# snayfach/MIDAS

Hardware: AMD Instinct MI355X
Metric: genomic sites/sec pileup+allele-count (higher is better)
Workload: dtype u8/u32 integer tallies (fp64 only in the two keep_read ratio tests)

## Files before the change

### midas_amd/build.py

```python

import concurrent.futures
import os
import shutil
import subprocess
import sys

HERE = os.path.dirname(os.path.abspath(__file__))
CSRC = os.path.join(HERE, "csrc")
LIB_DIR = os.path.join(HERE, "lib")
OBJ_DIR = os.path.join(LIB_DIR, "obj")
LIB_NAME = "libmidas_snps_hip.so"
LIB_PATH = os.path.join(LIB_DIR, LIB_NAME)

SOURCES = ["contigs.cpp", "bgzf_host.cpp", "bam_host.cpp", "bam_shares.cpp", "bam_writer.cpp", "tables_host.cpp", "fasta_host.cpp", "row_deflate.cpp", "comm.cpp", "pack_reads.hip", "index_reads.hip", "pileup_tiles.hip", "index_direct.hip", "pileup_direct.hip", "pileup_long.hip", "rows_deflate.hip", "bgzf_inflate.hip", "bam_walk.hip", "measure.hip", "merge_sites.hip", "merge_rows.hip", "tables_scan.hip", "tables_device.hip", "genes_count.hip", "genes_merge_io.cpp", "genes_merge.hip", "sites_io.cpp", "sites_scan.hip", "sites_strains.hip", "sites_trees.hip", "sites_pairs.hip", "sites_ld.hip", "nj_tree.hip", "genes_compare.hip", "genes_linkage.hip", "sam_scan.hip", "species_hits.hip", "species_assign.cpp", "species_merge.hip", "device_sort.hip", "mt19937_stream.hip", "bam_device.hip", "ctx_runtime.hip", "batch.hip", "batch_direct.hip", "batch_packed.hip", "batch_rows.hip"]
HEADERS = ["layout.h", "contigs.h", "kernels.h", "device_common.h", "pileup_common.h", "direct_common.h", "dense_bases.h", "ctx_internal.h", "batch.h", "filter_tables.h", "work_plan.h", "hostio.h", "hostio_internal.h", "bam_parse.h", "bam_record.h", "decode_plan.h", "sam_resident_plan.h", "tables_plan.h", "row_deflate.h", "workers.h", "crc32.h", "text_numbers.h", "text_rows.h", "bit_planes.h", "row_group_plan.h", "genes_rows.h", "sites_rows.h", "sites_call.h", "sites_resample.h", "draw_plan.h", "pandas_f64.h", "merge_fmt.h", "merge_rows.h", os.path.join("..", "..", "include", "midas_snps.h")]

FLAGS = ["--offload-arch=gfx950", "-O3", "-std=c++17", "-fPIC", "-mllvm", "-amdgpu-atomic-optimizer-strategy=None"]
SOURCE_FLAGS = {"sites_scan.hip": ["-ffp-contract=off"], "sites_strains.hip": ["-ffp-contract=off"], "sites_trees.hip": ["-ffp-contract=off"], "sites_pairs.hip": ["-ffp-contract=off"], "sites_ld.hip": ["-ffp-contract=off"],
                "genes_compare.hip": ["-ffp-contract=off"], "species_hits.hip": ["-ffp-contract=off"],
                "species_assign.cpp": ["-ffp-contract=off"], "species_merge.hip": ["-ffp-contract=off"], "merge_rows.hip": ["-ffp-contract=off"], "nj_tree.hip": ["-ffp-contract=off"]}


def _hipcc():
    for cand in (os.environ.get("HIPCC"), shutil.which("hipcc"), "/opt/rocm/bin/hipcc"):
        if cand and os.path.exists(cand):
            return cand
    raise RuntimeError("hipcc not found: cannot build %s" % LIB_NAME)


def _sources():
    return [s for s in SOURCES if os.path.exists(os.path.join(CSRC, s))]


def _newest_header():
    t = 0.0
    for h in HEADERS:
        p = os.path.join(CSRC, h)
        if os.path.exists(p):
            t = max(t, os.path.getmtime(p))
    return max(t, os.path.getmtime(os.path.abspath(__file__)))


def _stale():
    if not os.path.exists(LIB_PATH):
        return True
    t = os.path.getmtime(LIB_PATH)
    if _newest_header() > t:
        return True
    return any(os.path.getmtime(os.path.join(CSRC, s)) > t for s in _sources())


def _compile(obj, cmd, verbose):
    tmp = obj + ".tmp.%d" % os.getpid()
    try:
        _run(cmd + [tmp], verbose)
        os.replace(tmp, obj)
    finally:
        if os.path.exists(tmp):
            os.unlink(tmp)


def _run(cmd, verbose):
    if verbose:
        print(" ".join(cmd), file=sys.stderr)
    res = subprocess.run(cmd, stdout=subprocess.PIPE, stderr=subprocess.STDOUT, text=True)
    if res.returncode != 0:
        raise RuntimeError("hipcc failed (%d): %s\n%s" % (res.returncode, " ".join(cmd), res.stdout))


def build_native(force=False, verbose=False, extra_flags=(), lib_path=None, replace=None):
    variant = bool(extra_flags) or lib_path is not None or bool(replace)
    out = lib_path or LIB_PATH
    if not force and not variant and not _stale():
        return out
    hipcc = _hipcc()
    obj_dir = OBJ_DIR if not variant else OBJ_DIR + ".variant.%d" % os.getpid()
    os.makedirs(obj_dir, exist_ok=True)
    hdr_t = _newest_header()
    jobs = []
    objs = []
    for s in _sources():
        src = os.path.abspath(replace[s]) if replace and s in replace else os.path.join(CSRC, s)
        obj = os.path.join(obj_dir, s.replace(".", "_") + ".o")
        objs.append(obj)
        if force or variant or not os.path.exists(obj) or os.path.getmtime(obj) < max(hdr_t, os.path.getmtime(src)):
            jobs.append((obj, [hipcc] + FLAGS + SOURCE_FLAGS.get(s, []) + list(extra_flags) + ["-I", CSRC, "-x", "hip", "-c", src, "-o"]))
    try:
        workers = max(1, min(len(jobs), (os.cpu_count() or 4)))
        if jobs:
            with concurrent.futures.ThreadPoolExecutor(max_workers=workers) as pool:
                for f in [pool.submit(_compile, o, j, verbose) for (o, j) in jobs]:
                    f.result()
        tmp = out + ".tmp.%d" % os.getpid()
        try:
            _run([hipcc, "--offload-arch=gfx950", "-shared", "-fPIC"] + objs + ["-o", tmp, "-lz", "-lpthread", "-ldl"], verbose)
            os.replace(tmp, out)
        finally:
            if os.path.exists(tmp):
                os.unlink(tmp)
    finally:
        if variant:
            shutil.rmtree(obj_dir, ignore_errors=True)
    return out


if __name__ == "__main__":
    args = [a for a in sys.argv[1:]]
    force = "--force" in args
    verbose = "-v" in args
    out = None
    extra = []
    repl = {}
    it = iter(a for a in args if a not in ("--force", "-v"))
    for a in it:
        if a == "-o":
            out = next(it)
        elif a == "--replace":
            k, v = next(it).split("=", 1)
            repl[k] = v
        else:
            extra.append(a)
    print(build_native(force=force, verbose=verbose, extra_flags=extra, lib_path=out, replace=repl))
```

### midas_amd/csrc/index_direct.hip

```cpp
#include "dense_bases.h"
#include "direct_common.h"

namespace midas {

using namespace dev;
using namespace direct;

namespace {

constexpr int kIdxBlock = 256;
#ifndef MIDAS_IDX_RUN
#define MIDAS_IDX_RUN 2048
#endif
constexpr int kIdxRun = MIDAS_IDX_RUN;

__device__ __forceinline__ int contig_of_read(const DirectIndexParams& p, int i) {
  int lo = 0, hi = p.n_contigs;
  while (lo < hi) {
    const int mid = (lo + hi) >> 1;
    if (p.contig_read_begin[mid] > i) hi = mid; else lo = mid + 1;
  }
  int c = lo - 1;
  c = c < 0 ? 0 : c;
  return c > p.n_contigs - 1 ? p.n_contigs - 1 : c;
}
struct ContigCursor {
  int c, begin, next_begin, tile_base, tile_end;
  long long clen;
  __device__ __forceinline__ void fetch(const DirectIndexParams& p) {
    begin = p.contig_read_begin[c];
    next_begin = p.contig_read_begin[c + 1];
    clen = p.contig_len[c];
    tile_base = p.contig_tile_base[c];
    tile_end = p.contig_tile_base[c + 1];
  }
  __device__ __forceinline__ void advance(const DirectIndexParams& p, int i) {
    if (i < next_begin || c + 1 >= p.n_contigs) return;
    while (c + 1 < p.n_contigs && i >= p.contig_read_begin[c + 1]) ++c;
    fetch(p);
  }
};

__device__ __forceinline__ unsigned long long block_sum(unsigned long long v, unsigned long long* lds4) {
  for (int d = 32; d >= 1; d >>= 1) v += __shfl_down(v, d);
  __syncthreads();
  if ((threadIdx.x & 63) == 0) lds4[threadIdx.x >> 6] = v;
  __syncthreads();
  return lds4[0] + lds4[1] + lds4[2] + lds4[3];
}
__device__ __forceinline__ unsigned long long block_max(unsigned long long v, unsigned long long* lds4) {
  for (int d = 32; d >= 1; d >>= 1) {
    const unsigned long long o = __shfl_down(v, d);
    v = o > v ? o : v;
  }
  __syncthreads();
  if ((threadIdx.x & 63) == 0) lds4[threadIdx.x >> 6] = v;
  __syncthreads();
  const unsigned long long a = lds4[0] > lds4[1] ? lds4[0] : lds4[1], b = lds4[2] > lds4[3] ? lds4[2] : lds4[3];
  return a > b ? a : b;
}

template <bool SORTED>
__global__ __launch_bounds__(kIdxBlock) void direct_ranges_kernel(DirectIndexParams p) {
  __shared__ int s_c0;
  if (blockIdx.x == 0) {
    for (int i = threadIdx.x; i < p.n_stat_words; i += kIdxBlock) p.stats[i] = 0ull;
    if (threadIdx.x == 0 && p.err) *p.err = kNoError;
  }
  for (int i = blockIdx.x * kIdxBlock + threadIdx.x; i < p.n_tiles; i += gridDim.x * kIdxBlock) {
    p.tbegin_next[i] = 0xFFFFFFFFu;
    p.tend_next[i] = 0u;
  }
  const long long lo = (long long)blockIdx.x * kIdxRun;
  const long long hi = lo + kIdxRun < (long long)p.n_reads ? lo + kIdxRun : (long long)p.n_reads;
  if (lo >= hi) return;
  (void)s_c0;
  ContigCursor cur;
  {
    const DirectBlockCursor bc = p.block_contig[blockIdx.x];
    cur.c = bc.c; cur.begin = bc.begin; cur.next_begin = bc.next_begin; cur.tile_base = bc.tile_base; cur.tile_end = bc.tile_end;
    cur.clen = bc.clen;
  }
  const int lane = threadIdx.x & 63;
  constexpr int U = kIdxRun / kIdxBlock;
  int32_t pos[U], before[U];
#pragma unroll
  for (int u = 0; u < U; ++u) {
    const long long ii = lo + (long long)u * kIdxBlock + threadIdx.x;
    const long long ic = ii < hi ? ii : hi - 1;
    pos[u] = p.pos[ic];
    before[u] = p.pos[ic > 0 ? ic - 1 : 0];
  }
#pragma unroll
  for (int u = 0; u < U; ++u) {
    const long long ii = lo + (long long)u * kIdxBlock + threadIdx.x;
    const bool valid = ii < hi;
    uint32_t key = 0xFFFFFFFEu;
    int ka = 0, kb = 0;
    if (valid) {
      const int i = (int)ii;
      cur.advance(p, i);
      const long long last = cur.clen - 1;
      long long pc = pos[u];
      pc = pc < 0 ? 0 : (pc > last ? last : pc);
      const long long pr = pc + p.reach < last ? pc + p.reach : last;
      ka = cur.tile_base + (int)(pc >> p.tile_shift);
      kb = cur.tile_base + (int)(pr >> p.tile_shift);
      if (SORTED) {
        const bool first_of_contig = i == cur.begin;
        long long pb = before[u];
        pb = pb < 0 ? 0 : (pb > last ? last : pb);
        const long long pbr = pb + p.reach < last ? pb + p.reach : last;
        const int ka0 = first_of_contig ? cur.tile_base : cur.tile_base + (int)(pb >> p.tile_shift);
        const int kb0 = first_of_contig ? cur.tile_base - 1 : cur.tile_base + (int)(pbr >> p.tile_shift);
        for (int t = ka0; t < ka; ++t) p.tend[t] = (uint32_t)i;
        for (int t = kb0 + 1; t <= kb; ++t) p.tbegin[t] = (uint32_t)i;
        if (i == cur.next_begin - 1)
          for (int t = ka; t < cur.tile_end; ++t) p.tend[t] = (uint32_t)i + 1u;
      } else {
        key = (uint32_t)ka;
      }
    }
    if (!SORTED) {
      const uint32_t key_before = __shfl_up(key, 1), key_after = __shfl_down(key, 1);
      if (valid) {
        const uint32_t i = (uint32_t)ii;
        if (lane == 0 || key_before != key) atomicMin(&p.tbegin[ka], i);
        if (lane == 63 || key_after != key) atomicMax(&p.tend[ka], i + 1u);
        for (int t = ka + 1; t <= kb; ++t) {
          atomicMin(&p.tbegin[t], i);
          atomicMax(&p.tend[t], i + 1u);
        }
      }
    }
  }
}

struct Fields {
  long long so, so1, qo, qo1, co, co1;
  int32_t pos, l, nm;
};
__device__ __forceinline__ Fields load_fields(const DirectIndexParams& p, long long i) {
  Fields f;
  f.so = p.seq_off[i]; f.so1 = p.seq_off[i + 1];
  f.qo = p.qual_off[i]; f.qo1 = p.qual_off[i + 1];
  f.co = p.cigar_off[i]; f.co1 = p.cigar_off[i + 1];
  f.pos = p.pos[i]; f.l = p.l_seq[i]; f.nm = p.nm[i];
  return f;
}
__device__ __forceinline__ bool bad_layout(const DirectIndexParams& p, const Fields& f) {
  const long long l = f.l;
  return l < 0 || f.co1 - f.co < 0 || f.co < 0 || f.so < 0 || f.qo < 0 || f.so1 - f.so < (l + 1) / 2 || f.qo1 - f.qo < l ||
         f.so1 > p.seq_bytes || f.qo1 > p.qual_bytes || f.co1 > p.n_cigar;
}

__global__ __launch_bounds__(kIdxBlock) void direct_facts_kernel(DirectIndexParams p) {
  __shared__ unsigned long long red[4];
  __shared__ int s_c0;
  const long long lo = (long long)blockIdx.x * kIdxRun;
  const long long hi = lo + kIdxRun < (long long)p.n_reads ? lo + kIdxRun : (long long)p.n_reads;
  if (threadIdx.x == 0 && lo < hi) {
    s_c0 = contig_of_read(p, (int)lo);
    ContigCursor c0;
    c0.c = s_c0;
    c0.fetch(p);
    DirectBlockCursor bc;
    bc.c = c0.c; bc.begin = c0.begin; bc.next_begin = c0.next_begin; bc.tile_base = c0.tile_base; bc.tile_end = c0.tile_end; bc.pad = 0;
    bc.clen = c0.clen;
    p.block_contig[blockIdx.x] = bc;
  }
  __syncthreads();
  unsigned long long alg = 0, status = kNoError;
  uint32_t maxl = 0, maxspan = 0, unsorted = 0, general = 0, n_long = 0, n_out = 0, maxcommon = 0;
  ContigCursor cur;
  if (lo < hi) {
    cur.c = s_c0;
    cur.fetch(p);
  }
  for (long long ii = lo + threadIdx.x; ii < hi; ii += kIdxBlock) {
    const int i = (int)ii;
    cur.advance(p, i);
    const Fields f = load_fields(p, ii);
    const long long l = f.l, nc = f.co1 - f.co;
    {
      const long long last = cur.clen - 1;
      long long pc = f.pos, pb = p.pos[i > 0 ? i - 1 : 0];
      pc = pc < 0 ? 0 : (pc > last ? last : pc);
      pb = pb < 0 ? 0 : (pb > last ? last : pb);
      if (i != cur.begin && pb > pc) unsorted = 1u;
    }
    if (bad_layout(p, f)) {
      const unsigned long long s = ((unsigned long long)i << 8) | kPackBadLayout;
      status = s < status ? s : status;
      continue;
    }
    alg += (unsigned long long)((l + 1) / 2 + l + 4 * nc + 16);
    maxl = (uint32_t)l > maxl ? (uint32_t)l : maxl;
    if (l > kMaxLSeq || nc > kMaxField16 || f.nm > kMaxField16) {
      n_long += 1u;
      continue;
    }
    CigarView cg;
    cg.load(p.rec ? reinterpret_cast<const uint32_t*>(p.payload + ((unsigned long long)p.rec[i].off8 << 3)) : p.cigar + f.co);
    unsigned long long span = 0;
    for_each_op(cg, (uint32_t)nc, [&](uint32_t, uint32_t v) {
      const uint32_t op = v & 15u;
      if (op_is_match(op) || op == OP_D || op == OP_N) span += (unsigned long long)(v >> 4);
      return true;
    });
    span = span > 0x3FFFFFFFull ? 0x3FFFFFFFull : span;
    maxspan = (uint32_t)span > maxspan ? (uint32_t)span : maxspan;
    if (span > (unsigned long long)p.overhang) {
      n_out += 1u;
      const long long last = cur.clen - 1;
      long long pc = f.pos;
      pc = pc < 0 ? 0 : (pc > last ? last : pc);
      long long e = (long long)f.pos + (long long)span - 1;
      e = e > last ? last : e;
      if (e >= pc) {
        const uint32_t ka = (uint32_t)cur.tile_base + (uint32_t)(pc >> p.tile_shift), kb = (uint32_t)cur.tile_base + (uint32_t)(e >> p.tile_shift);
        if (kb > ka) {
          const uint32_t slot = atomicAdd(p.n_outliers_listed, 1u);
          if (slot < p.outlier_cap) p.outliers[slot] = DirectOutlier{(uint32_t)i, ka + 1u, kb, 0u};
        }
        const long long tile_start = (pc >> p.tile_shift) << p.tile_shift;
        if (e - tile_start >= (long long)(1 << p.tile_shift) + p.overhang)
          for (uint32_t t = ka; t <= kb; ++t) p.tile_flag[t] = 1;
      }
    } else {
      maxcommon = (uint32_t)span > maxcommon ? (uint32_t)span : maxcommon;
    }
    ReadShape sh;
    const bool fast = (uint32_t)nc <= 4u && decode_shape(cg.c0, cg.c1, cg.c2, cg.c3, (uint32_t)nc, (uint32_t)l, &sh) && f.nm >= 0 &&
                      f.pos >= 0 && (long long)f.pos < cur.clen;
    general += fast ? 0u : 1u;
  }
  alg = block_sum(alg, red);
  const unsigned long long ngen = block_sum((unsigned long long)general, red);
  const unsigned long long nlong = block_sum((unsigned long long)n_long, red);
  const unsigned long long bmax = block_max((unsigned long long)maxl, red);
  const unsigned long long bspan = block_max((unsigned long long)maxspan, red);
  const unsigned long long bcommon = block_max((unsigned long long)maxcommon, red);
  const unsigned long long nout = block_sum((unsigned long long)n_out, red);
  const unsigned long long any_unsorted = block_max((unsigned long long)unsorted, red);
  const unsigned long long worst = ~block_max(~status, red);
  if (threadIdx.x == 0) {
    DirectFacts* f = p.facts + (blockIdx.x % kDirectFactSlots);
    if (alg) atomicAdd(&f->alg_bytes, alg);
    if (ngen) atomicAdd(&f->n_general, (uint32_t)ngen);
    if (nlong) atomicAdd(&f->n_long, (uint32_t)nlong);
    if (bmax) atomicMax(&f->max_l, (uint32_t)bmax);
    if (bspan) atomicMax(&f->max_span, (uint32_t)bspan);
    if (bcommon) atomicMax(&f->max_span_common, (uint32_t)bcommon);
    if (nout) atomicAdd(&f->n_outliers, (uint32_t)nout);
    if (any_unsorted) atomicOr(&f->unsorted, 1u);
    if (worst != kNoError) atomicMin(&f->status, worst);
  }
}

__device__ __forceinline__ uint32_t read_units(const DirectLayoutParams& p, long long i) {
  return direct_payload_units((uint32_t)p.l_seq[i], (uint32_t)(p.cigar_off[i + 1] - p.cigar_off[i]));
}

__global__ __launch_bounds__(kIdxBlock) void direct_layout_units_kernel(DirectLayoutParams p) {
  __shared__ unsigned long long red[4];
  const long long lo = (long long)blockIdx.x * kIdxRun;
  const long long hi = lo + kIdxRun < p.n_reads ? lo + kIdxRun : p.n_reads;
  unsigned long long u = 0;
  for (long long i = lo + threadIdx.x; i < hi; i += kIdxBlock) u += read_units(p, i);
  u = block_sum(u, red);
  if (threadIdx.x == 0) p.block_units[blockIdx.x] = u;
}

__global__ __launch_bounds__(kIdxBlock) void direct_layout_scan_kernel(unsigned long long* v, int n_blocks) {
  __shared__ unsigned long long part[kIdxBlock];
  __shared__ unsigned long long carry;
  if (threadIdx.x == 0) carry = 0ull;
  __syncthreads();
  for (int base = 0; base < n_blocks; base += kIdxBlock) {
    const int i = base + (int)threadIdx.x;
    const unsigned long long x = i < n_blocks ? v[i] : 0ull;
    part[threadIdx.x] = x;
    __syncthreads();
    for (int d = 1; d < kIdxBlock; d <<= 1) {
      const unsigned long long y = (int)threadIdx.x >= d ? part[threadIdx.x - d] : 0ull;
      __syncthreads();
      part[threadIdx.x] += y;
      __syncthreads();
    }
    const unsigned long long c = carry;
    if (i < n_blocks) v[i] = c + part[threadIdx.x] - x;
    __syncthreads();
    if (threadIdx.x == kIdxBlock - 1) carry = c + part[kIdxBlock - 1];
    __syncthreads();
  }
  if (threadIdx.x == 0) v[n_blocks] = carry;
}

typedef uint32_t lay_u32x4_a1 __attribute__((ext_vector_type(4), aligned(1)));
__device__ __forceinline__ void group_copy(uint8_t* dst, const uint8_t* src, uint32_t len, int gl) {
  for (uint32_t k = (uint32_t)gl * 16u; k < len; k += 256u) {
    if (k + 16u <= len) {
      *reinterpret_cast<lay_u32x4_a1*>(dst + k) = *reinterpret_cast<const lay_u32x4_a1*>(src + k);
    } else {
      for (uint32_t j = k; j < len; ++j) dst[j] = src[j];
    }
  }
}

__global__ __launch_bounds__(kIdxBlock) void direct_layout_fill_kernel(DirectLayoutParams p) {
  constexpr int U = kIdxRun / kIdxBlock;
  __shared__ uint32_t s_off[kIdxRun];
  __shared__ uint32_t s_part[kIdxBlock];
  const long long lo = (long long)blockIdx.x * kIdxRun;
  const long long hi = lo + kIdxRun < p.n_reads ? lo + kIdxRun : p.n_reads;
  const unsigned long long base = p.block_units[blockIdx.x];
  uint32_t units[U], sum = 0;
#pragma unroll
  for (int u = 0; u < U; ++u) {
    const long long i = lo + (long long)threadIdx.x * U + u;
    units[u] = i < hi ? read_units(p, i) : 0u;
    sum += units[u];
  }
  s_part[threadIdx.x] = sum;
  __syncthreads();
  for (int d = 1; d < kIdxBlock; d <<= 1) {
    const uint32_t y = (int)threadIdx.x >= d ? s_part[threadIdx.x - d] : 0u;
    __syncthreads();
    s_part[threadIdx.x] += y;
    __syncthreads();
  }
  uint32_t run = s_part[threadIdx.x] - sum;
#pragma unroll
  for (int u = 0; u < U; ++u) {
    const long long i = lo + (long long)threadIdx.x * U + u;
    s_off[threadIdx.x * U + u] = run;
    if (i < hi) {
      const int32_t nm = p.nm[i];
      DirectRec r;
      r.pos = p.pos[i];
      r.l_nc = (uint32_t)p.l_seq[i] | ((uint32_t)(p.cigar_off[i + 1] - p.cigar_off[i]) << 16);
      r.nmq = (nm < 0 ? (uint32_t)kNmAbsent : (uint32_t)nm) | ((uint32_t)p.mapq[i] << 16);
      r.off8 = (uint32_t)(base + run);
      p.rec[i] = r;
    }
    run += units[u];
  }
  if (blockIdx.x == gridDim.x - 1 && threadIdx.x == 0) {
    DirectRec r;
    r.pos = 0; r.l_nc = 0u; r.nmq = 0u; r.off8 = (uint32_t)(base + s_part[kIdxBlock - 1]);
    p.rec[p.n_reads] = r;
  }
  __syncthreads();
  const int grp = (int)(threadIdx.x >> 4), gl = (int)(threadIdx.x & 15);
  for (long long i = lo + grp; i < hi; i += kIdxBlock / 16) {
    const uint32_t l = (uint32_t)p.l_seq[i];
    const long long co = p.cigar_off[i];
    const uint32_t nc = (uint32_t)(p.cigar_off[i + 1] - co);
    uint8_t* dst = p.payload + 8ull * (base + s_off[(int)(i - lo)]);
    group_copy(dst, reinterpret_cast<const uint8_t*>(p.cigar + co), 4u * nc, gl);
    (void)dense::encode<16>(dst + 4u * nc, 8u * direct_payload_units(l, nc) - 4u * nc, p.seq4 + p.seq_off[i], p.qual + p.qual_off[i], l, gl, p.side);
  }
}

__global__ __launch_bounds__(256) void direct_outliers_kernel(const DirectOutlier* list, uint32_t n, uint32_t* tbegin) {
  const uint32_t j = blockIdx.x * 256u + threadIdx.x;
  if (j >= n) return;
  const DirectOutlier o = list[j];
  for (uint32_t t = o.t_first; t <= o.t_last; ++t) atomicMin(&tbegin[t], o.read);
}

}

hipError_t launch_direct_outliers(const DirectOutlier* list, uint32_t n, uint32_t* tbegin, hipStream_t s) {
  if (n == 0u) return hipSuccess;
  hipLaunchKernelGGL(direct_outliers_kernel, dim3((n + 255u) / 256u), dim3(256), 0, s, list, n, tbegin);
  return hipGetLastError();
}

int direct_index_blocks(int64_t n_reads) { return n_reads > 0 ? (int)((n_reads + kIdxRun - 1) / kIdxRun) : 1; }

hipError_t launch_direct_facts(const DirectIndexParams& p, hipStream_t s) {
  hipLaunchKernelGGL(direct_facts_kernel, dim3(direct_index_blocks(p.n_reads)), dim3(kIdxBlock), 0, s, p);
  return hipGetLastError();
}

hipError_t launch_direct_layout_sizes(const DirectLayoutParams& p, hipStream_t s) {
  const int nb = direct_index_blocks(p.n_reads);
  hipLaunchKernelGGL(direct_layout_units_kernel, dim3(nb), dim3(kIdxBlock), 0, s, p);
  hipLaunchKernelGGL(direct_layout_scan_kernel, dim3(1), dim3(kIdxBlock), 0, s, p.block_units, nb);
  return hipGetLastError();
}

hipError_t launch_direct_layout_fill(const DirectLayoutParams& p, hipStream_t s) {
  hipLaunchKernelGGL(direct_layout_fill_kernel, dim3(direct_index_blocks(p.n_reads)), dim3(kIdxBlock), 0, s, p);
  return hipGetLastError();
}

hipError_t launch_direct_ranges(const DirectIndexParams& p, hipStream_t s) {
  const int grid = direct_index_blocks(p.n_reads);
  if (p.sorted) hipLaunchKernelGGL(direct_ranges_kernel<true>, dim3(grid), dim3(kIdxBlock), 0, s, p);
  else hipLaunchKernelGGL(direct_ranges_kernel<false>, dim3(grid), dim3(kIdxBlock), 0, s, p);
  return hipGetLastError();
}

}
```

Baseline: 114.4 billion.

## Restructure sorted tile-range indexing with vectorized lane-contiguous loads and ballot-skipped stores

The sorted path of the direct ranges kernel is rewritten so each lane owns four consecutive reads, loaded with a single 16-byte vector load. The previous read's position now comes from a cross-lane shuffle instead of a second global load. Wave-uniform contig fields are hoisted with readfirstlane when a block covers a single contig. A wave ballot skips the store loops when no lane has tile boundaries to publish, and the tile math moves to 32-bit arithmetic. The intent is to cut redundant global loads and divergent per-read work in a small indexing pre-pass, at the cost of more complex lane geometry and an extra head-element load per group.

Result: slower. 110.8 billion (-3.1%).

```diff
diff --git a/midas_amd/build.py b/midas_amd/build.py
--- a/midas_amd/build.py
+++ b/midas_amd/build.py
@@ -13,7 +13,7 @@
 LIB_PATH = os.path.join(LIB_DIR, LIB_NAME)
 
 SOURCES = ["contigs.cpp", "bgzf_host.cpp", "bam_host.cpp", "bam_shares.cpp", "bam_writer.cpp", "tables_host.cpp", "fasta_host.cpp", "row_deflate.cpp", "comm.cpp", "pack_reads.hip", "index_reads.hip", "pileup_tiles.hip", "index_direct.hip", "pileup_direct.hip", "pileup_long.hip", "rows_deflate.hip", "bgzf_inflate.hip", "bam_walk.hip", "measure.hip", "merge_sites.hip", "merge_rows.hip", "tables_scan.hip", "tables_device.hip", "genes_count.hip", "genes_merge_io.cpp", "genes_merge.hip", "sites_io.cpp", "sites_scan.hip", "sites_strains.hip", "sites_trees.hip", "sites_pairs.hip", "sites_ld.hip", "nj_tree.hip", "genes_compare.hip", "genes_linkage.hip", "sam_scan.hip", "species_hits.hip", "species_assign.cpp", "species_merge.hip", "device_sort.hip", "mt19937_stream.hip", "bam_device.hip", "ctx_runtime.hip", "batch.hip", "batch_direct.hip", "batch_packed.hip", "batch_rows.hip"]
-HEADERS = ["layout.h", "contigs.h", "kernels.h", "device_common.h", "pileup_common.h", "direct_common.h", "dense_bases.h", "ctx_internal.h", "batch.h", "filter_tables.h", "work_plan.h", "hostio.h", "hostio_internal.h", "bam_parse.h", "bam_record.h", "decode_plan.h", "sam_resident_plan.h", "tables_plan.h", "row_deflate.h", "workers.h", "crc32.h", "text_numbers.h", "text_rows.h", "bit_planes.h", "row_group_plan.h", "genes_rows.h", "sites_rows.h", "sites_call.h", "sites_resample.h", "draw_plan.h", "pandas_f64.h", "merge_fmt.h", "merge_rows.h", os.path.join("..", "..", "include", "midas_snps.h")]
+HEADERS = ["layout.h", "contigs.h", "kernels.h", "device_common.h", "pileup_common.h", "direct_common.h", "ranges_tiles.h", "dense_bases.h", "ctx_internal.h", "batch.h", "filter_tables.h", "work_plan.h", "hostio.h", "hostio_internal.h", "bam_parse.h", "bam_record.h", "decode_plan.h", "sam_resident_plan.h", "tables_plan.h", "row_deflate.h", "workers.h", "crc32.h", "text_numbers.h", "text_rows.h", "bit_planes.h", "row_group_plan.h", "genes_rows.h", "sites_rows.h", "sites_call.h", "sites_resample.h", "draw_plan.h", "pandas_f64.h", "merge_fmt.h", "merge_rows.h", os.path.join("..", "..", "include", "midas_snps.h")]
 
 FLAGS = ["--offload-arch=gfx950", "-O3", "-std=c++17", "-fPIC", "-mllvm", "-amdgpu-atomic-optimizer-strategy=None"]
 SOURCE_FLAGS = {"sites_scan.hip": ["-ffp-contract=off"], "sites_strains.hip": ["-ffp-contract=off"], "sites_trees.hip": ["-ffp-contract=off"], "sites_pairs.hip": ["-ffp-contract=off"], "sites_ld.hip": ["-ffp-contract=off"],
diff --git a/midas_amd/csrc/index_direct.hip b/midas_amd/csrc/index_direct.hip
--- a/midas_amd/csrc/index_direct.hip
+++ b/midas_amd/csrc/index_direct.hip
@@ -1,5 +1,6 @@
 #include "dense_bases.h"
 #include "direct_common.h"
+#include "ranges_tiles.h"
 
 namespace midas {
 
@@ -9,10 +10,12 @@
 namespace {
 
 constexpr int kIdxBlock = 256;
-#ifndef MIDAS_IDX_RUN
-#define MIDAS_IDX_RUN 2048
+
+#ifdef MIDAS_ISA_MARKS
+#define MIDAS_MARK(name) asm volatile("; MARK " name)
+#else
+#define MIDAS_MARK(name) do { } while (0)
 #endif
-constexpr int kIdxRun = MIDAS_IDX_RUN;
 
 __device__ __forceinline__ int contig_of_read(const DirectIndexParams& p, int i) {
   int lo = 0, hi = p.n_contigs;
@@ -60,9 +63,7 @@
   return a > b ? a : b;
 }
 
-template <bool SORTED>
-__global__ __launch_bounds__(kIdxBlock) void direct_ranges_kernel(DirectIndexParams p) {
-  __shared__ int s_c0;
+__device__ __forceinline__ void reset_for_the_next_run(const DirectIndexParams& p) {
   if (blockIdx.x == 0) {
     for (int i = threadIdx.x; i < p.n_stat_words; i += kIdxBlock) p.stats[i] = 0ull;
     if (threadIdx.x == 0 && p.err) *p.err = kNoError;
@@ -71,10 +72,121 @@
     p.tbegin_next[i] = 0xFFFFFFFFu;
     p.tend_next[i] = 0u;
   }
+}
+
+constexpr int kLaneReads = kRangesLaneReads;
+constexpr int kGroupReads = kIdxBlock * kLaneReads;
+constexpr int kGroups = kIdxRun / kGroupReads;
+static_assert(kRangesWaveReads == 64 * kLaneReads && kGroups * kGroupReads == kIdxRun && kLaneReads == 4, "lane geometry of the sorted ranges pass");
+typedef int32_t pos_x4 __attribute__((ext_vector_type(4), aligned(4)));
+
+template <bool ONE_CONTIG>
+__device__ __forceinline__ void sorted_groups(const DirectIndexParams& p, ContigCursor cur, int lo, int n, const int32_t (&pos)[kGroups][kLaneReads],
+                                              const int32_t (&head)[kGroups]) {
+  const int lane = threadIdx.x & 63;
+  int32_t last = (int32_t)(cur.clen - 1);
+  if (ONE_CONTIG) {
+    cur.begin = __builtin_amdgcn_readfirstlane(cur.begin); cur.next_begin = __builtin_amdgcn_readfirstlane(cur.next_begin);
+    cur.tile_base = __builtin_amdgcn_readfirstlane(cur.tile_base); cur.tile_end = __builtin_amdgcn_readfirstlane(cur.tile_end);
+    last = __builtin_amdgcn_readfirstlane(last);
+  }
+#pragma unroll
+  for (int g = 0; g < kGroups; ++g) {
+    MIDAS_MARK("group");
+    const int rel0 = g * kGroupReads + (int)threadIdx.x * kLaneReads;
+    const int32_t below = __shfl_up(pos[g][kLaneReads - 1], 1);
+    const int32_t before = lane == 0 ? head[g] : below;
+    int ka[kLaneReads], kb[kLaneReads], ka0[kLaneReads], kb0[kLaneReads], kend[kLaneReads];
+    bool publish[kLaneReads], any = false;
+    ReadTiles prev{0, 0};
+#pragma unroll
+    for (int k = 0; k < kLaneReads; ++k) {
+      const bool valid = rel0 + k < n;
+      const int i = lo + rel0 + k;
+#ifdef MIDAS_RANGES_FLOOR
+      ka[k] = kb[k] = ka0[k] = kb0[k] = kend[k] = 0;
+      publish[k] = valid && pos[g][k] == INT32_MIN && before == INT32_MAX && i == last;
+      (void)prev;
+#else
+      if (!ONE_CONTIG && valid) {
+        cur.advance(p, i);
+        last = (int32_t)(cur.clen - 1);
+      }
+      if (k == 0) prev = read_tiles(before, last, p.reach, p.tile_shift, cur.tile_base);
+      const ReadTiles t = read_tiles(pos[g][k], last, p.reach, p.tile_shift, cur.tile_base);
+      const bool first_of_contig = i == cur.begin;
+      ka[k] = t.start; kb[k] = t.reach;
+      ka0[k] = first_of_contig ? cur.tile_base : prev.start;
+      kb0[k] = first_of_contig ? cur.tile_base - 1 : prev.reach;
+      kend[k] = i == cur.next_begin - 1 ? cur.tile_end : t.start;
+      publish[k] = valid && (ka0[k] < ka[k] || kb0[k] < kb[k] || i == cur.next_begin - 1);
+      prev = t;
+#endif
+      any = any || publish[k];
+    }
+    MIDAS_MARK("ballot");
+    if (__ballot(any) == 0ull) continue;
+    MIDAS_MARK("stores");
+#pragma unroll
+    for (int k = 0; k < kLaneReads; ++k) {
+      if (!publish[k]) continue;
+      const uint32_t i = (uint32_t)(lo + rel0 + k);
+      for (int t = ka0[k]; t < ka[k]; ++t) p.tend[t] = i;
+      for (int t = kb0[k] + 1; t <= kb[k]; ++t) p.tbegin[t] = i;
+      for (int t = ka[k]; t < kend[k]; ++t) p.tend[t] = i + 1u;
+    }
+  }
+  MIDAS_MARK("group");
+}
+
+__device__ __forceinline__ void ranges_sorted(const DirectIndexParams& p) {
+  const int lo = (int)blockIdx.x * kIdxRun;
+  const int n = p.n_reads - lo < kIdxRun ? p.n_reads - lo : kIdxRun;
+  if (n <= 0) {
+    reset_for_the_next_run(p);
+    return;
+  }
+  MIDAS_MARK("loads");
+  const int32_t* src = p.pos + lo;
+  int32_t pos[kGroups][kLaneReads], head[kGroups];
+  if (n == kIdxRun) {
+#pragma unroll
+    for (int g = 0; g < kGroups; ++g) {
+      const pos_x4 v = *reinterpret_cast<const pos_x4*>(src + g * kGroupReads + (int)threadIdx.x * kLaneReads);
+#pragma unroll
+      for (int k = 0; k < kLaneReads; ++k) pos[g][k] = v[k];
+    }
+  } else {
+#pragma unroll
+    for (int g = 0; g < kGroups; ++g)
+#pragma unroll
+      for (int k = 0; k < kLaneReads; ++k) {
+        const int rel = g * kGroupReads + (int)threadIdx.x * kLaneReads + k;
+        pos[g][k] = src[rel < n ? rel : n - 1];
+      }
+  }
+  const int wave = __builtin_amdgcn_readfirstlane((int)(threadIdx.x >> 6));
+#pragma unroll
+  for (int g = 0; g < kGroups; ++g) {
+    int h = g * kGroupReads + wave * kRangesWaveReads - 1;
+    h = h < n - 1 ? h : n - 1;
+    h = h > -lo ? h : -lo;
+    head[g] = src[h];
+  }
+  const DirectBlockCursor bc = p.block_contig[blockIdx.x];
+  reset_for_the_next_run(p);
+  ContigCursor cur;
+  cur.c = bc.c; cur.begin = bc.begin; cur.next_begin = bc.next_begin; cur.tile_base = bc.tile_base; cur.tile_end = bc.tile_end;
+  cur.clen = bc.clen;
+  if (cur.next_begin >= lo + n) sorted_groups<true>(p, cur, lo, n, pos, head);
+  else sorted_groups<false>(p, cur, lo, n, pos, head);
+}
+
+__device__ __forceinline__ void ranges_unsorted(const DirectIndexParams& p) {
+  reset_for_the_next_run(p);
   const long long lo = (long long)blockIdx.x * kIdxRun;
   const long long hi = lo + kIdxRun < (long long)p.n_reads ? lo + kIdxRun : (long long)p.n_reads;
   if (lo >= hi) return;
-  (void)s_c0;
   ContigCursor cur;
   {
     const DirectBlockCursor bc = p.block_contig[blockIdx.x];
@@ -83,13 +195,11 @@
   }
   const int lane = threadIdx.x & 63;
   constexpr int U = kIdxRun / kIdxBlock;
-  int32_t pos[U], before[U];
+  int32_t pos[U];
 #pragma unroll
   for (int u = 0; u < U; ++u) {
     const long long ii = lo + (long long)u * kIdxBlock + threadIdx.x;
-    const long long ic = ii < hi ? ii : hi - 1;
-    pos[u] = p.pos[ic];
-    before[u] = p.pos[ic > 0 ? ic - 1 : 0];
+    pos[u] = p.pos[ii < hi ? ii : hi - 1];
   }
 #pragma unroll
   for (int u = 0; u < U; ++u) {
@@ -98,30 +208,16 @@
     uint32_t key = 0xFFFFFFFEu;
     int ka = 0, kb = 0;
     if (valid) {
-      const int i = (int)ii;
-      cur.advance(p, i);
+      cur.advance(p, (int)ii);
       const long long last = cur.clen - 1;
       long long pc = pos[u];
       pc = pc < 0 ? 0 : (pc > last ? last : pc);
       const long long pr = pc + p.reach < last ? pc + p.reach : last;
       ka = cur.tile_base + (int)(pc >> p.tile_shift);
       kb = cur.tile_base + (int)(pr >> p.tile_shift);
-      if (SORTED) {
-        const bool first_of_contig = i == cur.begin;
-        long long pb = before[u];
-        pb = pb < 0 ? 0 : (pb > last ? last : pb);
-        const long long pbr = pb + p.reach < last ? pb + p.reach : last;
-        const int ka0 = first_of_contig ? cur.tile_base : cur.tile_base + (int)(pb >> p.tile_shift);
-        const int kb0 = first_of_contig ? cur.tile_base - 1 : cur.tile_base + (int)(pbr >> p.tile_shift);
-        for (int t = ka0; t < ka; ++t) p.tend[t] = (uint32_t)i;
-        for (int t = kb0 + 1; t <= kb; ++t) p.tbegin[t] = (uint32_t)i;
-        if (i == cur.next_begin - 1)
-          for (int t = ka; t < cur.tile_end; ++t) p.tend[t] = (uint32_t)i + 1u;
-      } else {
-        key = (uint32_t)ka;
-      }
-    }
-    if (!SORTED) {
+      key = (uint32_t)ka;
+    }
+    {
       const uint32_t key_before = __shfl_up(key, 1), key_after = __shfl_down(key, 1);
       if (valid) {
         const uint32_t i = (uint32_t)ii;
@@ -134,6 +230,12 @@
       }
     }
   }
+}
+
+template <bool SORTED>
+__global__ __launch_bounds__(kIdxBlock) void direct_ranges_kernel(DirectIndexParams p) {
+  if (SORTED) ranges_sorted(p);
+  else ranges_unsorted(p);
 }
 
 struct Fields {
diff --git a/midas_amd/csrc/ranges_tiles.h b/midas_amd/csrc/ranges_tiles.h
--- /dev/null
+++ b/midas_amd/csrc/ranges_tiles.h
@@ -0,0 +1,28 @@
+#pragma once
+#include <cstdint>
+
+#if defined(__HIPCC__) || defined(__CUDACC__)
+#define MIDAS_RANGES_HD __host__ __device__ __forceinline__
+#else
+#define MIDAS_RANGES_HD inline
+#endif
+
+namespace midas {
+
+#ifndef MIDAS_IDX_RUN
+#define MIDAS_IDX_RUN 2048
+#endif
+constexpr int kIdxRun = MIDAS_IDX_RUN;
+constexpr int kRangesLaneReads = 4;
+constexpr int kRangesWaveReads = 256;
+
+struct ReadTiles { int32_t start, reach; };
+
+MIDAS_RANGES_HD ReadTiles read_tiles(int32_t pos, int32_t last, int32_t reach, int32_t tile_shift, int32_t tile_base) {
+  const int32_t pc = pos < 0 ? 0 : (pos > last ? last : pos);
+  const uint32_t sum = (uint32_t)pc + (uint32_t)reach;
+  const uint32_t pr = sum < (uint32_t)last ? sum : (uint32_t)last;
+  return ReadTiles{tile_base + (int32_t)((uint32_t)pc >> tile_shift), tile_base + (int32_t)(pr >> tile_shift)};
+}
+
+}
```
